# TheStageAI/TheWhisper

Hardware: NVIDIA H100
Metric: tokens_per_sec (higher is better)
Workload: dtype bf16

## Files before the change

include/thewhisper_b200.h:

```cpp
#ifndef THEWHISPER_B200_H_
#define THEWHISPER_B200_H_

#include <stddef.h>
#include <stdint.h>

#ifdef __cplusplus
extern "C" {
#endif

#define BW_ABI_VERSION 2

typedef struct bw_engine bw_engine;

#ifndef THEWHISPER_B200_TYPES_
#define THEWHISPER_B200_TYPES_
typedef struct bw_config {
  int32_t d_model;
  int32_t n_heads;
  int32_t ffn;
  int32_t enc_layers;
  int32_t dec_layers;
  int32_t n_mels;
  int32_t vocab;
  int32_t max_source_positions;
// ... 52 lines not shown
int bw_word_timestamps_batch(bw_engine* e, int32_t n, const int32_t* audio, const int32_t* n_tokens, const int32_t* num_frames,
                             double time_precision, float* out_host, int32_t out_pitch, void* stream);
int bw_word_timestamps_gather(bw_engine* e, int32_t n, const int32_t* slot_map, int32_t map_pitch, const int32_t* n_tokens,
                              const int32_t* num_frames, double time_precision, float* out_host, int32_t out_pitch, void* stream);

int bw_host_merge_overlapping(const int32_t* tokens, const int32_t* lens, int32_t n_seq, const double* ts,
                              int32_t* out_tokens, double* out_ts, int32_t* out_len);

typedef struct bw_host_vocab bw_host_vocab;
int bw_host_vocab_create(const uint8_t* bytes, const int64_t* offsets, int32_t n_vocab, const int32_t* kind, const char* language_names,
                         int32_t n_languages, int32_t timestamp_begin, int32_t render_begin, int32_t eos_id, int32_t sot_id,
                         int32_t startofprev_id, int32_t cleanup_spaces, bw_host_vocab** out);
void bw_host_vocab_destroy(bw_host_vocab* v);
int bw_host_decode_asr(bw_host_vocab* v, const int32_t* tokens, const int32_t* lens, int32_t n_out, const double* token_ts, const int32_t* ts_lens,
                       const double* strides, const uint8_t* has_stride, int32_t mode, int32_t return_language, double time_precision,
                       int32_t default_language, const char** json_out, int64_t* json_len);

int bw_op_gemm(const void* A, const void* W, int32_t M, int32_t N, int32_t K, const float* bias, float alpha, int32_t act,
               const float* residual, void* out, int32_t out_is_f32, int32_t impl, int32_t force_bn, void* stream);
int bw_op_gemm_splitk(const void* A, const void* W, int32_t M, int32_t N, int32_t K, int32_t n_valid, int32_t ksplit, int32_t force_bn,
                      float* out_partials, int32_t* ksplit_used, void* stream);
int bw_op_gemm_dec(const void* X, const void* W, int32_t Q, int32_t N, int32_t K, int32_t n_valid, int32_t want_split, float* out_partials,
                   int32_t* ksplit_used, void* stream);
int bw_op_gelu_bias(const float* partials, int32_t nsplit, const float* bias, void* h_bf16, int32_t Q, int32_t N, void* stream);
int bw_op_resid_ln(float* x, const float* partials, int32_t nsplit, const float* bias, const float* ln_g, const float* ln_b, void* y_bf16,
                   int32_t Q, int32_t D, void* stream);
int bw_op_attn_enc(const void* qkv, void* vt_scratch, void* out, int32_t B, int32_t S, int32_t H, int32_t impl, void* stream);
int bw_op_layernorm(const float* x, const float* g, const float* b, void* out, int32_t out_is_f32, int32_t rows, int32_t D,
                    void* stream);
int bw_op_gemv(const float* x, const float* ln_g, const float* ln_b, const void* W, int32_t M, int32_t N, int32_t K,
               const float* bias, float alpha, int32_t act, const float* residual, float* out, void* stream);
int bw_op_mega_plan(int32_t Q, int32_t D, int32_t ffn, int32_t num_sms, int32_t smem_optin, int32_t static_smem, int64_t* out);
int bw_op_mega_plan_w8(int32_t Q, int32_t D, int32_t ffn, int32_t num_sms, int32_t smem_optin, int32_t static_smem, int64_t* out);

#ifdef __cplusplus
}
#endif
#endif
```

thewhisper_b200/_lib.py:

```python
from __future__ import annotations

import ctypes as C
import os
from typing import Optional

_HERE = os.path.dirname(os.path.abspath(__file__))
LIB_PATH = os.path.join(_HERE, "_C", "libthewhisper_b200.so")


class BwError(RuntimeError):
    pass


class bw_config(C.Structure):
    _fields_ = [(n, C.c_int32) for n in (
        "d_model", "n_heads", "ffn", "enc_layers", "dec_layers", "n_mels", "vocab", "max_source_positions",
        "max_target_positions", "max_audios", "max_beams", "n_align_heads", "max_align_steps", "dtype")]


class bw_decode_opts(C.Structure):
    _fields_ = [
        ("begin_index", C.c_int32), ("eos_token", C.c_int32), ("pad_token", C.c_int32),
        ("timestamp_rules", C.c_int32), ("timestamp_begin", C.c_int32), ("no_timestamps_token", C.c_int32),
        ("max_initial_timestamp_index", C.c_int32),
# ... 20 lines not shown
    "bw_engine_buffer": (C.c_int, [_P, C.c_char_p, C.POINTER(_P), C.POINTER(C.c_size_t)]),
    "bw_logmel": (C.c_int, [_P, _P, _I, _I, _P, _P]),
    "bw_logmel_long": (C.c_int, [_P, _P, _I, _I, _P, _P]),
    "bw_set_mel": (C.c_int, [_P, _P, _I, _P]),
    "bw_encode": (C.c_int, [_P, _I, _P]),
    "bw_decode_begin": (C.c_int, [_P, _I, _I, _P, _I, C.POINTER(bw_decode_opts), _P]),
    "bw_decode_begin_key_start": (C.c_int, [_P, _I, _I, _P, _I, C.POINTER(bw_decode_opts), _P, _P]),
    "bw_decode_run": (C.c_int, [_P, _I, _P]),
    "bw_decode_prefill": (C.c_int, [_P, _I, _I, _P]),
    "bw_decode_kernel_launches": (C.c_longlong, [_P]),
    "bw_decode_graph_stats": (C.c_int, [_P, C.POINTER(C.c_int64)]),
    "bw_decode_read": (C.c_int, [_P, _P, _P, _P, _P]),
    "bw_decode_scores_enable": (C.c_int, [_P, _I, _I, _P]),
    "bw_decode_read_scores": (C.c_int, [_P, _P, _P, _P, _P]),
    "bw_decode_reorder": (C.c_int, [_P, _P, _P, _P]),
    "bw_decode_beam_step": (C.c_int, [_P, _P, _P, _P, _P]),
    "bw_word_timestamps": (C.c_int, [_P, _I, _I, _I, C.c_double, _P, _P]),
    "bw_word_timestamps_batch": (C.c_int, [_P, _I, _P, _P, _P, C.c_double, _P, _I, _P]),
    "bw_word_timestamps_gather": (C.c_int, [_P, _I, _P, _I, _P, _P, C.c_double, _P, _I, _P]),
    "bw_host_merge_overlapping": (C.c_int, [_P, _P, _I, _P, _P, _P, _P]),
    "bw_host_vocab_create": (C.c_int, [_P, _P, _I, _P, C.c_char_p, _I, _I, _I, _I, _I, _I, _I, _P]),
    "bw_host_vocab_destroy": (None, [_P]),
    "bw_host_decode_asr": (C.c_int, [_P, _P, _P, _I, _P, _P, _P, _P, _I, _I, C.c_double, _I, _P, _P]),
    "bw_op_gemm": (C.c_int, [_P, _P, _I, _I, _I, _P, _F, _I, _P, _P, _I, _I, _I, _P]),
    "bw_op_gemm_splitk": (C.c_int, [_P, _P, _I, _I, _I, _I, _I, _I, _P, C.POINTER(_I), _P]),
    "bw_op_gemm_dec": (C.c_int, [_P, _P, _I, _I, _I, _I, _I, _P, C.POINTER(_I), _P]),
    "bw_op_gelu_bias": (C.c_int, [_P, _I, _P, _P, _I, _I, _P]),
    "bw_op_resid_ln": (C.c_int, [_P, _P, _I, _P, _P, _P, _P, _I, _I, _P]),
    "bw_op_attn_enc": (C.c_int, [_P, _P, _P, _I, _I, _I, _I, _P]),
    "bw_op_layernorm": (C.c_int, [_P, _P, _P, _P, _I, _I, _I, _P]),
    "bw_op_gemv": (C.c_int, [_P, _P, _P, _P, _I, _I, _I, _P, _F, _I, _P, _P, _P]),
    "bw_op_mega_plan": (C.c_int, [_I, _I, _I, _I, _I, _I, C.POINTER(C.c_int64)]),
    "bw_op_mega_plan_w8": (C.c_int, [_I, _I, _I, _I, _I, _I, C.POINTER(C.c_int64)]),
}

_lib: Optional[C.CDLL] = None


def load(build_if_missing: bool = False) -> C.CDLL:
    global _lib
    if _lib is not None:
        return _lib
    if not os.path.exists(LIB_PATH):
        if build_if_missing:
            from . import build as _build

            _build.build()
        else:
            raise BwError(f"{LIB_PATH} not found: run `python -m thewhisper_b200.build` (nvcc, sm_90a). "
                          "thewhisper_b200 has no CPU fallback.")
    lib = C.CDLL(LIB_PATH)
    for name, (res, args) in SYMBOLS.items():
        fn = getattr(lib, name)
        fn.restype = res
        fn.argtypes = args
    if lib.bw_abi_version() != 2:
        raise BwError("ABI version mismatch")
    _lib = lib
    return lib


def check(rc: int) -> None:
    if rc != 0:
        msg = load().bw_last_error()
        raise BwError((msg or b"unknown error").decode("utf-8", "replace") + f" (code {rc})")

# ... 14 lines not shown
```

thewhisper_b200/csrc/abi.cu:

```cuda
#include "../../include/thewhisper_b200.h"

#define BW_RENAME_SUFFIX _bf16
#include "abi_rename.h"
#undef THEWHISPER_B200_H_
#include "../../include/thewhisper_b200.h"
#include "abi_unrename.h"
#undef BW_CAT
#undef BW_CAT2
#define BW_RENAME_SUFFIX _f16
#include "abi_rename.h"
#undef THEWHISPER_B200_H_
#include "../../include/thewhisper_b200.h"
#include "abi_unrename.h"

struct bw_engine {
  int f16;
  void* impl;
};

namespace {
thread_local int g_last_f16 = 0;
}
#define BW_B(e) reinterpret_cast<bw_engine_bf16*>((e)->impl)
#define BW_H(e) reinterpret_cast<bw_engine_f16*>((e)->impl)
// ... 108 lines not shown
  g_last_f16 = 0;
  return bw_op_gemm_dec_bf16(X, W, Q, N, K, n_valid, want_split, out_partials, ksplit_used, stream);
}
int bw_op_gelu_bias(const float* partials, int32_t nsplit, const float* bias, void* h_bf16, int32_t Q, int32_t N, void* stream) {
  g_last_f16 = 0;
  return bw_op_gelu_bias_bf16(partials, nsplit, bias, h_bf16, Q, N, stream);
}
int bw_op_resid_ln(float* x, const float* partials, int32_t nsplit, const float* bias, const float* ln_g, const float* ln_b, void* y_bf16,
                   int32_t Q, int32_t D, void* stream) {
  g_last_f16 = 0;
  return bw_op_resid_ln_bf16(x, partials, nsplit, bias, ln_g, ln_b, y_bf16, Q, D, stream);
}
int bw_op_attn_enc(const void* qkv, void* vt_scratch, void* out, int32_t B, int32_t S, int32_t H, int32_t impl, void* stream) {
  g_last_f16 = 0;
  return bw_op_attn_enc_bf16(qkv, vt_scratch, out, B, S, H, impl, stream);
}
int bw_op_layernorm(const float* x, const float* g, const float* b, void* out, int32_t out_is_f32, int32_t rows, int32_t D, void* stream) {
  g_last_f16 = 0;
  return bw_op_layernorm_bf16(x, g, b, out, out_is_f32, rows, D, stream);
}
int bw_op_gemv(const float* x, const float* ln_g, const float* ln_b, const void* W, int32_t M, int32_t N, int32_t K, const float* bias,
               float alpha, int32_t act, const float* residual, float* out, void* stream) {
  g_last_f16 = 0;
  return bw_op_gemv_bf16(x, ln_g, ln_b, W, M, N, K, bias, alpha, act, residual, out, stream);
}
int bw_op_mega_plan(int32_t Q, int32_t D, int32_t ffn, int32_t num_sms, int32_t smem_optin, int32_t static_smem, int64_t* out) {
  g_last_f16 = 0;
  return bw_op_mega_plan_bf16(Q, D, ffn, num_sms, smem_optin, static_smem, out);
}
int bw_op_mega_plan_w8(int32_t Q, int32_t D, int32_t ffn, int32_t num_sms, int32_t smem_optin, int32_t static_smem, int64_t* out) {
  g_last_f16 = 0;
  return bw_op_mega_plan_w8_bf16(Q, D, ffn, num_sms, smem_optin, static_smem, out);
}

}
```

thewhisper_b200/csrc/abi_rename.h:

```cpp
#define BW_CAT2(a, b) a##b
#define BW_CAT(a, b) BW_CAT2(a, b)
#define bw_engine BW_CAT(bw_engine, BW_RENAME_SUFFIX)
#define bw_last_error BW_CAT(bw_last_error, BW_RENAME_SUFFIX)
#define bw_abi_version BW_CAT(bw_abi_version, BW_RENAME_SUFFIX)
#define bw_device_count BW_CAT(bw_device_count, BW_RENAME_SUFFIX)
#define bw_runtime_flags BW_CAT(bw_runtime_flags, BW_RENAME_SUFFIX)
#define bw_engine_create BW_CAT(bw_engine_create, BW_RENAME_SUFFIX)
#define bw_engine_destroy BW_CAT(bw_engine_destroy, BW_RENAME_SUFFIX)
#define bw_engine_set_tensor BW_CAT(bw_engine_set_tensor, BW_RENAME_SUFFIX)
#define bw_engine_set_mel_filters BW_CAT(bw_engine_set_mel_filters, BW_RENAME_SUFFIX)
#define bw_engine_set_alignment_heads BW_CAT(bw_engine_set_alignment_heads, BW_RENAME_SUFFIX)
#define bw_engine_finalize BW_CAT(bw_engine_finalize, BW_RENAME_SUFFIX)
#define bw_engine_buffer BW_CAT(bw_engine_buffer, BW_RENAME_SUFFIX)
#define bw_logmel BW_CAT(bw_logmel, BW_RENAME_SUFFIX)
#define bw_logmel_long BW_CAT(bw_logmel_long, BW_RENAME_SUFFIX)
#define bw_set_mel BW_CAT(bw_set_mel, BW_RENAME_SUFFIX)
#define bw_encode BW_CAT(bw_encode, BW_RENAME_SUFFIX)
#define bw_decode_begin BW_CAT(bw_decode_begin, BW_RENAME_SUFFIX)
#define bw_decode_begin_key_start BW_CAT(bw_decode_begin_key_start, BW_RENAME_SUFFIX)
#define bw_decode_run BW_CAT(bw_decode_run, BW_RENAME_SUFFIX)
#define bw_decode_prefill BW_CAT(bw_decode_prefill, BW_RENAME_SUFFIX)
#define bw_decode_graph_stats BW_CAT(bw_decode_graph_stats, BW_RENAME_SUFFIX)
#define bw_decode_kernel_launches BW_CAT(bw_decode_kernel_launches, BW_RENAME_SUFFIX)
#define bw_decode_read BW_CAT(bw_decode_read, BW_RENAME_SUFFIX)
#define bw_decode_scores_enable BW_CAT(bw_decode_scores_enable, BW_RENAME_SUFFIX)
#define bw_decode_read_scores BW_CAT(bw_decode_read_scores, BW_RENAME_SUFFIX)
#define bw_decode_reorder BW_CAT(bw_decode_reorder, BW_RENAME_SUFFIX)
#define bw_decode_beam_step BW_CAT(bw_decode_beam_step, BW_RENAME_SUFFIX)
#define bw_word_timestamps BW_CAT(bw_word_timestamps, BW_RENAME_SUFFIX)
#define bw_word_timestamps_batch BW_CAT(bw_word_timestamps_batch, BW_RENAME_SUFFIX)
#define bw_op_gemm BW_CAT(bw_op_gemm, BW_RENAME_SUFFIX)
#define bw_op_gemm_splitk BW_CAT(bw_op_gemm_splitk, BW_RENAME_SUFFIX)
#define bw_op_gemm_dec BW_CAT(bw_op_gemm_dec, BW_RENAME_SUFFIX)
#define bw_op_gelu_bias BW_CAT(bw_op_gelu_bias, BW_RENAME_SUFFIX)
#define bw_op_resid_ln BW_CAT(bw_op_resid_ln, BW_RENAME_SUFFIX)
#define bw_op_attn_enc BW_CAT(bw_op_attn_enc, BW_RENAME_SUFFIX)
#define bw_op_layernorm BW_CAT(bw_op_layernorm, BW_RENAME_SUFFIX)
#define bw_op_gemv BW_CAT(bw_op_gemv, BW_RENAME_SUFFIX)
#define bw_op_mega_plan BW_CAT(bw_op_mega_plan, BW_RENAME_SUFFIX)
#define bw_op_mega_plan_w8 BW_CAT(bw_op_mega_plan_w8, BW_RENAME_SUFFIX)
#define bw_word_timestamps_gather BW_CAT(bw_word_timestamps_gather, BW_RENAME_SUFFIX)
```

thewhisper_b200/csrc/abi_unrename.h:

```cpp
#undef bw_engine
#undef bw_last_error
#undef bw_abi_version
#undef bw_device_count
#undef bw_runtime_flags
#undef bw_engine_create
#undef bw_engine_destroy
#undef bw_engine_set_tensor
#undef bw_engine_set_mel_filters
#undef bw_engine_set_alignment_heads
#undef bw_engine_finalize
#undef bw_engine_buffer
#undef bw_logmel
#undef bw_logmel_long
#undef bw_set_mel
#undef bw_encode
#undef bw_decode_begin
#undef bw_decode_begin_key_start
#undef bw_decode_run
#undef bw_decode_prefill
#undef bw_decode_kernel_launches
#undef bw_decode_graph_stats
#undef bw_decode_read
#undef bw_decode_scores_enable
#undef bw_decode_read_scores
#undef bw_decode_reorder
#undef bw_decode_beam_step
#undef bw_word_timestamps
#undef bw_word_timestamps_batch
#undef bw_op_gemm
#undef bw_op_gemm_splitk
#undef bw_op_gemm_dec
#undef bw_op_gelu_bias
#undef bw_op_resid_ln
#undef bw_op_attn_enc
#undef bw_op_layernorm
#undef bw_op_gemv
#undef bw_op_mega_plan
#undef bw_op_mega_plan_w8
#undef bw_word_timestamps_gather
#undef BW_RENAME_SUFFIX
```

thewhisper_b200/csrc/api.cu:

```cuda
#include <limits.h>
#include <stdarg.h>
#include <stdlib.h>
#include <string.h>

#include <chrono>
#include <map>
#include <string>
#include <tuple>
#include <vector>

#ifdef BW_F16
#define BW_RENAME_SUFFIX _f16
#define BW_API_NS bw_api_f16
#else
#define BW_RENAME_SUFFIX _bf16
#define BW_API_NS bw_api
#endif
#include "abi_rename.h"
#include "../../include/thewhisper_b200.h"
#include "decode.cuh"
#include "decode_mega_common.cuh"
#include "kernels.h"

namespace BW_NS {
// ... 1231 lines not shown
int bw_op_layernorm(const float* x, const float* g, const float* b, void* out, int32_t out_is_f32, int32_t rows, int32_t D, void* stream) {
  BW_CHECK(x && g && b && out, "bw_op_layernorm: null pointer");
  cudaStream_t st = static_cast<cudaStream_t>(stream);
  return out_is_f32 ? layernorm_f32(st, x, g, b, static_cast<float*>(out), rows, D)
                    : layernorm_bf16(st, x, g, b, static_cast<bf16*>(out), rows, D);
}

int bw_op_gemv(const float* x, const float* ln_g, const float* ln_b, const void* W, int32_t M, int32_t N, int32_t K, const float* bias,
               float alpha, int32_t act, const float* residual, float* out, void* stream) {
  BW_CHECK(x && W && out, "bw_op_gemv: null pointer");
  GemvArgs g;
  g.x = x; g.ldx = K; g.ln_g = ln_g; g.ln_b = ln_b; g.W = static_cast<const bf16*>(W); g.N = N; g.K = K; g.M = M;
  g.bias = bias; g.alpha = alpha; g.alpha_cols = (alpha != 1.0f) ? N : 0; g.act = act; g.residual = residual; g.out = out; g.ldo = N;
  return launch_gemv(static_cast<cudaStream_t>(stream), g);
}

static int mega_plan(int32_t Q, int32_t D, int32_t ffn, int32_t num_sms, int32_t smem_optin, int32_t static_smem, int64_t* out, int esz) {
  BW_CHECK(out && Q >= 1 && D > 0 && ffn > 0 && num_sms > 0 && smem_optin > static_smem, "bw_op_mega_plan: bad arguments");
  int p0_off = 0;
  const size_t smem = mega::mega_smem_plan(Q <= 1 ? 1 : 2, D, ffn, num_sms, true, (size_t)(smem_optin - static_smem), &p0_off, esz);
  out[0] = (int64_t)smem;
  out[1] = p0_off;
  return smem ? 0 : -3;
}

int bw_op_mega_plan(int32_t Q, int32_t D, int32_t ffn, int32_t num_sms, int32_t smem_optin, int32_t static_smem, int64_t* out) {
  return mega_plan(Q, D, ffn, num_sms, smem_optin, static_smem, out, 2);
}

int bw_op_mega_plan_w8(int32_t Q, int32_t D, int32_t ffn, int32_t num_sms, int32_t smem_optin, int32_t static_smem, int64_t* out) {
  return mega_plan(Q, D, ffn, num_sms, smem_optin, static_smem, out, 1);
}

}
```

thewhisper_b200/csrc/gemm_tc.cu:

```cuda
#include <limits.h>

#include "kernels.h"

namespace BW_NS {

namespace {

constexpr int BM = 128;
constexpr int BK = 64;
constexpr int A_STAGE_BYTES = BM * BK * 2;
constexpr int THREADS = 288;
constexpr int CONSUMER_WARPS = 8;

template <int BN>
struct Cfg {
  static constexpr int STAGES = (BN == 256) ? 4 : (BN == 128) ? 6 : 8;
  static constexpr int B_STAGE_BYTES = BN * BK * 2;
  static constexpr int SMEM_BYTES = STAGES * (A_STAGE_BYTES + B_STAGE_BYTES) + 1024  + 256 ;
};

enum { EPI_GENERIC = 0, EPI_GELU = 1 , EPI_RESID = 2 , EPI_PLAIN = 3  };

struct GemmParams {
  int B, rows, N, K;
  int rows_per_item = INT_MAX;
  int fast_gelu = 0;
  int kwrap;
  int tiles_m;
  int ksplit;
  int kper;
  long long split_stride;
  GemmEpi epi;
};

__device__ __forceinline__ void tma_load_3d(void* smem_dst, const CUtensorMap* m, uint64_t* bar, int c0, int c1, int c2) {
  asm volatile(
      "cp.async.bulk.tensor.3d.shared::cluster.global.mbarrier::complete_tx::bytes [%0], [%1, {%3, %4, %5}], [%2];" ::"r"(
          smem_u32(smem_dst)),
      "l"(reinterpret_cast<uint64_t>(m)), "r"(smem_u32(bar)), "r"(c0), "r"(c1), "r"(c2)
      : "memory");
}

__device__ __forceinline__ float gelu_as(float x) {
  const float ax = fabsf(x);
  float t;
  asm("rcp.approx.ftz.f32 %0, %1;" : "=f"(t) : "f"(fmaf(0.3275911f * 0.70710678f, ax, 1.0f)));
  float q = 0.5f * 1.061405429f;
  q = fmaf(q, t, 0.5f * -1.453152027f);
  q = fmaf(q, t, 0.5f * 1.421413741f);
  q = fmaf(q, t, 0.5f * -0.284496736f);
  q = fmaf(q, t, 0.5f * 0.254829592f);
  q = (q * t) * ex2_approx((x * -0.72134752f) * x);
  return fmaf(-ax, q, fmaxf(x, 0.f));
}

template <int BN, int MODE>
__global__ void __launch_bounds__(THREADS, 1)
gemm_tc_kernel(const __grid_constant__ CUtensorMap tmA, const __grid_constant__ CUtensorMap tmW, const GemmParams p) {
  using C = Cfg<BN>;
  extern __shared__ uint8_t smem_raw[];
  uint8_t* smem = reinterpret_cast<uint8_t*>((reinterpret_cast<uintptr_t>(smem_raw) + 1023) & ~uintptr_t(1023));
  uint8_t* sA = smem;
  uint8_t* sB = smem + C::STAGES * A_STAGE_BYTES;
  uint64_t* bars = reinterpret_cast<uint64_t*>(sB + C::STAGES * C::B_STAGE_BYTES);
  uint64_t* full = bars;
  uint64_t* empty = bars + C::STAGES;

  const int warp = threadIdx.x >> 5;
  const int lane = threadIdx.x & 31;
  const int b = blockIdx.y / p.tiles_m;
  const int t0 = (blockIdx.y % p.tiles_m) * BM;
  const int n0 = blockIdx.x * BN;
  const int nk_all = (p.K + BK - 1) / BK;
  const int kb0 = (int)blockIdx.z * p.kper;
  const int nk = min(nk_all, kb0 + p.kper) - kb0;

  if (threadIdx.x == 0) {
    for (int s = 0; s < C::STAGES; ++s) {
      mbar_init(&full[s], 1);
      mbar_init(&empty[s], CONSUMER_WARPS);
    }
    fence_mbar_init();
  }
  if (warp == CONSUMER_WARPS && lane == 0) {
    tma_prefetch_desc(&tmA);
    tma_prefetch_desc(&tmW);
  }
  __syncthreads();

// ... 6 lines not shown
      }
      pdl_wait();
      pdl_launch();
      for (int kb = 0; kb < nk; ++kb) {
        const int s = kb % C::STAGES;
        const uint32_t ph = (kb / C::STAGES) & 1;
        const int k = (kb0 + kb) * BK;
        if (kb >= npre) {
          mbar_wait_wg(&empty[s], ph ^ 1);
          mbar_arrive_expect_tx(&full[s], A_STAGE_BYTES + C::B_STAGE_BYTES);
          tma_load_2d(sB + s * C::B_STAGE_BYTES, &tmW, &full[s], k, n0);
        }
        tma_load_3d(sA + s * A_STAGE_BYTES, &tmA, &full[s], k % p.kwrap, t0 + k / p.kwrap, b);
      }
    }
  } else {
    const int g = warp >> 2;
    float acc[BN / 2];
#pragma unroll
    for (int i = 0; i < BN / 2; ++i) acc[i] = 0.f;
    for (int kb = 0; kb < nk; ++kb) {
      const int s = kb % C::STAGES;
      mbar_wait_wg(&full[s], (kb / C::STAGES) & 1);
      wg_fence();
      wg_kblock<BN>(acc, smem_u32(sA + s * A_STAGE_BYTES + g * (A_STAGE_BYTES / 2)), smem_u32(sB + s * C::B_STAGE_BYTES));
      wg_commit();
      wg_wait<1>();
      if (kb > 0 && lane == 0) mbar_arrive(&empty[(kb - 1) % C::STAGES]);
    }
    wg_wait<0>();
    wg_pin(acc);

    pdl_wait();
    const GemmEpi& e = p.epi;
    constexpr bool GEN = MODE == EPI_GENERIC;
    const bool do_alpha = GEN && e.alpha != 1.0f;
    const bool do_act = GEN ? e.act == 1 : MODE == EPI_GELU;
    const bool fast_gelu = GEN ? p.fast_gelu != 0 : true;
    const bool has_pos = GEN && e.pos != nullptr;
    const bool has_res = GEN ? e.residual != nullptr : MODE == EPI_RESID;
    const bool f32out = GEN ? e.out_f32 != nullptr : MODE == EPI_RESID;
    const int r = g * 64 + (warp & 3) * 16 + (lane >> 2);
#pragma unroll
    for (int h = 0; h < 2; ++h) {
      const int t = t0 + r + 8 * h;
      if (t >= p.rows) continue;
      const int bi = t / p.rows_per_item, ti = t - bi * p.rows_per_item;
      const long long row_off = (long long)(b + bi) * e.batch_stride + (long long)ti * e.row_stride + (long long)blockIdx.z * p.split_stride;
#pragma unroll
      for (int j = 0; j < BN / 8; ++j) {
        const int n = n0 + 8 * j + 2 * (lane & 3);
        if (n >= p.N) break;
        float f0 = acc[4 * j + 2 * h], f1 = acc[4 * j + 2 * h + 1];
        if (e.bias) {
          const float2 bb = __ldg(reinterpret_cast<const float2*>(e.bias + n));
          f0 += bb.x; f1 += bb.y;
        }
        if (do_alpha && n < e.alpha_cols) { f0 *= e.alpha; f1 *= e.alpha; }
        if (do_act) {
          if (fast_gelu) { f0 = gelu_as(f0); f1 = gelu_as(f1); }
          else { f0 = gelu_erf(f0); f1 = gelu_erf(f1); }
        }
        if (has_pos) {
          const float2 q = *reinterpret_cast<const float2*>(e.pos + (long long)t * p.N + n);
          f0 += q.x; f1 += q.y;
        }
        const long long off = row_off + (long long)(n >> 6) * e.head_stride + (n & 63);
        if (has_res) {
          const float2 q = *reinterpret_cast<const float2*>(e.residual + off);
          f0 += q.x; f1 += q.y;
        }
        if (f32out) *reinterpret_cast<float2*>(e.out_f32 + off) = make_float2(f0, f1);
        else *reinterpret_cast<uint32_t*>(e.out_bf16 + off) = pack_bf16(f0, f1);
      }
    }
  }
}

__global__ void gemm_simt_kernel(GemmA a, const bf16* __restrict__ W, GemmParams p) {
  const int n = blockIdx.x * 16 + threadIdx.x;
  const int t = (blockIdx.y % p.tiles_m) * 16 + threadIdx.y;
  const int b = blockIdx.y / p.tiles_m;
  if (n >= p.N || t >= p.rows) return;
  const bf16* ab = a.base + (long long)b * a.batch_stride;
  const bf16* w = W + (long long)n * p.K;
  float acc = 0.f;
  const int kend = (p.epi.n_valid > 0 && n >= p.epi.n_valid) ? 0 : p.K;
  for (int k = 0; k < kend; ++k) {
    const float av = e2f(ab[(long long)(t + k / p.kwrap) * a.pitch + (k % p.kwrap)]);
    acc = fmaf(av, e2f(w[k]), acc);
  }
  const GemmEpi& e = p.epi;
  const long long off = (long long)b * e.batch_stride + (long long)t * e.row_stride + (long long)(n >> 6) * e.head_stride + (n & 63);
  if (e.bias) acc += e.bias[n];
  if (n < e.alpha_cols) acc *= e.alpha;
  if (e.act == 1) acc = gelu_erf(acc);
  if (e.pos) acc += e.pos[(long long)t * p.N + n];
  if (e.residual) acc += e.residual[off];
  if (e.out_f32) e.out_f32[off] = acc;
  else e.out_bf16[off] = f2e(acc);
}

typedef CUresult (*EncodeTiledFn)(CUtensorMap*, CUtensorMapDataType, cuuint32_t, void*, const cuuint64_t*, const cuuint64_t*,
                                  const cuuint32_t*, const cuuint32_t*, CUtensorMapInterleave, CUtensorMapSwizzle,
                                  CUtensorMapL2promotion, CUtensorMapFloatOOBfill);

EncodeTiledFn get_encode_fn() {
// ... 115 lines not shown
  GemmParams p;
  p.B = B; p.rows = rows; p.N = N; p.K = K;
  p.kwrap = a.kwrap >= K ? INT_MAX : a.kwrap;
  p.tiles_m = (rows + BM - 1) / BM;
  p.epi = epi;
  {
    const int nk = K / BK;
    p.ksplit = gemm_tc_ksplit(K, ksplit);
    p.kper = (nk + p.ksplit - 1) / p.ksplit;
    p.split_stride = split_stride;
  }
  const uint64_t inner = (uint64_t)(a.kwrap >= K ? K : a.kwrap);
  CUtensorMap tmA;
  if (int rc = make_tmap_3d_bf16(&tmA, a.base, (uint64_t)B, (uint64_t)a.rows_base, inner, (uint64_t)a.pitch * 2,
                                 (uint64_t)(B > 1 ? a.batch_stride : (long long)a.rows_base * a.pitch) * 2, BM, BK))
    return rc;
  int bn = force_bn;
  if (bn == 0) {
    const long long tiles128 = (long long)((N + 127) / 128) * p.tiles_m * B;
    bn = (N % 256 == 0 && tiles128 >= 4 * device_sms()) ? 256 : 128;
    if (N < 128) bn = 64;
  }
  switch (bn) {
    case 32: return launch_tc<32>(st, tmA, W, p);
    case 64: return launch_tc<64>(st, tmA, W, p);
    case 128: return launch_tc<128>(st, tmA, W, p);
    case 256: return launch_tc<256>(st, tmA, W, p);
  }
  BW_CHECK(false, "gemm_tc: unsupported BN=%d", bn);
}

bool gemm_tc2_supported(int M, int N, int K) { return K % BK == 0 && K >= BK && (N % 256 == 0 || N % 128 == 0) && M >= 1; }

int gemm_tc2(cudaStream_t st, const bf16* A, const bf16* W, int M, int N, int K, int rows_per_item, const GemmEpi& epi, int force_bn) {
  BW_CHECK((epi.out_f32 != nullptr) != (epi.out_bf16 != nullptr), "gemm_tc2: exactly one of out_f32/out_bf16 must be set");
  BW_CHECK(gemm_tc2_supported(M, N, K), "gemm_tc2: unsupported shape M=%d N=%d K=%d", M, N, K);
  BW_CHECK(!epi.pos, "gemm_tc2: positional-table epilogue is not supported (conv stem stays on gemm_tc)");
  BW_CHECK(epi.row_stride % 8 == 0 && epi.batch_stride % 8 == 0 && epi.head_stride % 8 == 0, "gemm_tc2: output strides must be multiples of 8");
  GemmParams p;
  p.B = 1; p.rows = M; p.N = N; p.K = K;
  p.rows_per_item = rows_per_item > 0 ? rows_per_item : INT_MAX;
  p.fast_gelu = 1;
  p.kwrap = INT_MAX;
  p.tiles_m = (M + BM - 1) / BM;
  p.ksplit = 1; p.kper = K / BK; p.split_stride = 0;
  p.epi = epi;
  CUtensorMap tmA;
  if (int rc = make_tmap_3d_bf16(&tmA, A, 1, (uint64_t)M, (uint64_t)K, (uint64_t)K * 2, (uint64_t)M * K * 2, BM, BK)) return rc;
  int force_mode = -1;
  if (force_bn >= 1000) {
    force_mode = EPI_GENERIC;
    force_bn -= 1000;
  }
  int bn = force_bn;
  if (bn == 0) {
    bn = (N % 256 == 0) ? 256 : 128;
    if (bn == 256) {
      const int sms = device_sms();
      const long long t256 = (long long)p.tiles_m * (N / 256);
      const long long waves = (t256 + sms - 1) / sms;
      if (t256 * 10 < waves * sms * 8) bn = 128;
    }
  }
  BW_CHECK(bn == 128 || bn == 256, "gemm_tc2: unsupported tile width %d", bn);
  BW_CHECK(N % bn == 0, "gemm_tc2: N=%d is not a multiple of the tile width %d", N, bn);
  int mode = EPI_GENERIC;
  if (epi.alpha == 1.0f) {
    if (epi.act == 1 && !epi.residual && epi.out_bf16) mode = EPI_GELU;
    else if (epi.act == 0 && epi.residual && epi.out_f32) mode = EPI_RESID;
    else if (epi.act == 0 && !epi.residual && epi.out_bf16) mode = EPI_PLAIN;
  }
  if (force_mode >= 0) mode = force_mode;
#define BW_TC2_CASE(BNV, MODEV) \
  if (bn == BNV && mode == MODEV) return launch_tc<BNV, MODEV>(st, tmA, W, p);
  BW_TC2_CASE(256, EPI_GENERIC) BW_TC2_CASE(256, EPI_GELU) BW_TC2_CASE(256, EPI_RESID) BW_TC2_CASE(256, EPI_PLAIN)
  BW_TC2_CASE(128, EPI_GENERIC) BW_TC2_CASE(128, EPI_GELU) BW_TC2_CASE(128, EPI_RESID) BW_TC2_CASE(128, EPI_PLAIN)
#undef BW_TC2_CASE
  BW_CHECK(false, "gemm_tc2: no kernel for bn=%d mode=%d", bn, mode);
}

int gemm_simt(cudaStream_t st, const GemmA& a, const bf16* W, int B, int rows, int N, int K, const GemmEpi& epi) {
  if (int rc = check_epi(epi, N)) return rc;
  GemmParams p;
  p.B = B; p.rows = rows; p.N = N; p.K = K;
  p.kwrap = a.kwrap >= K ? INT_MAX : a.kwrap;
  p.tiles_m = (rows + 15) / 16;
  p.ksplit = 1; p.kper = 0; p.split_stride = 0;
  p.epi = epi;
  dim3 grid((N + 15) / 16, p.tiles_m * B);
  gemm_simt_kernel<<<grid, dim3(16, 16), 0, st>>>(a, W, p);
  BW_CUDA_OK(cudaGetLastError());
  return 0;
}

}
```

thewhisper_b200/csrc/kernels.h:

```cpp
#pragma once
#include "common.cuh"

namespace BW_NS {

struct GemmA {
  const bf16* base = nullptr;
  long long batch_stride = 0;
  long long pitch = 0;
  int rows_base = 0;
  int kwrap = 0x7fffffff;
};

struct GemmEpi {
  const float* bias = nullptr;
  float alpha = 1.0f;
  int alpha_cols = 0x7fffffff;
  int act = 0;
  const float* residual = nullptr;
  const float* pos = nullptr;
  float* out_f32 = nullptr;
  bf16* out_bf16 = nullptr;
  long long batch_stride = 0;
  long long row_stride = 0;
  long long head_stride = 64;
  int n_valid = 0;
};

int gemm_tc(cudaStream_t st, const GemmA& a, const bf16* W, int B, int rows, int N, int K, const GemmEpi& epi,
            int force_bn );
int gemm_tc_split(cudaStream_t st, const GemmA& a, const bf16* W, int B, int rows, int N, int K, const GemmEpi& epi, int force_bn,
                  int ksplit, long long split_stride);
int gemm_tc_ksplit(int K, int ksplit);
bool gemm_tc2_supported(int M, int N, int K);
int gemm_tc2(cudaStream_t st, const bf16* A, const bf16* W, int M, int N, int K, int rows_per_item, const GemmEpi& epi, int force_bn);
int gemm_simt(cudaStream_t st, const GemmA& a, const bf16* W, int B, int rows, int N, int K, const GemmEpi& epi);

struct DecGemmPlan {
  int QB = 16, q_tiles = 1, stages = 2, kper = 1, ksplit = 1;
  size_t smem = 0;
};
DecGemmPlan gemm_dec_plan(int Q, int N, int K, int num_sms, bool want_split, bool w8 = false);
int gemm_dec(cudaStream_t st, const bf16* X, const void* W, const float* wscale, int Q, int N, int K, int n_valid, const GemmEpi& epi,
             const DecGemmPlan& pl, long long split_stride);
int launch_gelu_bias(cudaStream_t st, const float* part, int nsplit, long long split_stride, const float* bias, bf16* h, int Q, int N);

int attn_enc_tc(cudaStream_t st, const bf16* qkv, const bf16* vt, bf16* out, int B, int S, int Spad, int H);
int attn_enc_simt(cudaStream_t st, const bf16* qkv, bf16* out, int B, int S, int H);
int transpose_v(cudaStream_t st, const bf16* qkv, bf16* vt, int B, int S, int Spad, int H);

int layernorm_bf16(cudaStream_t st, const float* x, const float* g, const float* b, bf16* y, int rows, int D);
int layernorm_f32(cudaStream_t st, const float* x, const float* g, const float* b, float* y, int rows, int D);

struct LogmelPlan;
int logmel_plan_create_from_bank(LogmelPlan** out, const float* bank , int n_mels);
void logmel_plan_destroy(LogmelPlan* p);
int logmel(cudaStream_t st, const LogmelPlan* plan, const float* pcm, int B, int n_samples, int frames, bf16* out_tm,
           float* out_f32, float* scratch, unsigned* scratch_max);
int logmel_long(cudaStream_t st, const LogmelPlan* plan, const float* pcm, int B, int n_samples, float* out_f32, unsigned* scratch_max);

}
```

Before: 845.3.

## Make tc2 GEMM persistent with ping-pong warpgroups and a shared tile planner

Replaces the one-CTA-per-tile tc2 launch with a persistent kernel capped at the SM count that loops over tiles. When there are enough 128-wide tiles and K is small, it schedules two consumer warpgroups in ping-pong so one group's epilogue overlaps the other's MMA. The epilogue is factored out and now prefetches residuals in batches, and tile selection moves into a plan function exposed through the ABI. The aims are to cut launch and tail-wave waste and hide epilogue cost, at the price of more complex barrier logic and possible load imbalance.

```diff
diff --git a/include/thewhisper_b200.h b/include/thewhisper_b200.h
--- a/include/thewhisper_b200.h
+++ b/include/thewhisper_b200.h
@@ -108,6 +108,8 @@
                const float* bias, float alpha, int32_t act, const float* residual, float* out, void* stream);
 int bw_op_mega_plan(int32_t Q, int32_t D, int32_t ffn, int32_t num_sms, int32_t smem_optin, int32_t static_smem, int64_t* out);
 int bw_op_mega_plan_w8(int32_t Q, int32_t D, int32_t ffn, int32_t num_sms, int32_t smem_optin, int32_t static_smem, int64_t* out);
+int bw_op_gemm_tc2_plan(int32_t M, int32_t N, int32_t K, int32_t num_sms, int32_t* out);
+int bw_op_gemm_tc2_tiles(int32_t M, int32_t N, int32_t K, int32_t num_sms, int32_t* out, int32_t cap);
 
 #ifdef __cplusplus
 }
diff --git a/thewhisper_b200/_lib.py b/thewhisper_b200/_lib.py
--- a/thewhisper_b200/_lib.py
+++ b/thewhisper_b200/_lib.py
@@ -76,6 +76,8 @@
     "bw_op_gemv": (C.c_int, [_P, _P, _P, _P, _I, _I, _I, _P, _F, _I, _P, _P, _P]),
     "bw_op_mega_plan": (C.c_int, [_I, _I, _I, _I, _I, _I, C.POINTER(C.c_int64)]),
     "bw_op_mega_plan_w8": (C.c_int, [_I, _I, _I, _I, _I, _I, C.POINTER(C.c_int64)]),
+    "bw_op_gemm_tc2_plan": (C.c_int, [_I, _I, _I, _I, C.POINTER(_I)]),
+    "bw_op_gemm_tc2_tiles": (C.c_int, [_I, _I, _I, _I, C.POINTER(_I), _I]),
 }
 
 _lib: Optional[C.CDLL] = None
diff --git a/thewhisper_b200/csrc/abi.cu b/thewhisper_b200/csrc/abi.cu
--- a/thewhisper_b200/csrc/abi.cu
+++ b/thewhisper_b200/csrc/abi.cu
@@ -164,5 +164,13 @@
   g_last_f16 = 0;
   return bw_op_mega_plan_w8_bf16(Q, D, ffn, num_sms, smem_optin, static_smem, out);
 }
+int bw_op_gemm_tc2_plan(int32_t M, int32_t N, int32_t K, int32_t num_sms, int32_t* out) {
+  g_last_f16 = 0;
+  return bw_op_gemm_tc2_plan_bf16(M, N, K, num_sms, out);
+}
+int bw_op_gemm_tc2_tiles(int32_t M, int32_t N, int32_t K, int32_t num_sms, int32_t* out, int32_t cap) {
+  g_last_f16 = 0;
+  return bw_op_gemm_tc2_tiles_bf16(M, N, K, num_sms, out, cap);
+}
 
 }
diff --git a/thewhisper_b200/csrc/abi_rename.h b/thewhisper_b200/csrc/abi_rename.h
--- a/thewhisper_b200/csrc/abi_rename.h
+++ b/thewhisper_b200/csrc/abi_rename.h
@@ -39,4 +39,6 @@
 #define bw_op_gemv BW_CAT(bw_op_gemv, BW_RENAME_SUFFIX)
 #define bw_op_mega_plan BW_CAT(bw_op_mega_plan, BW_RENAME_SUFFIX)
 #define bw_op_mega_plan_w8 BW_CAT(bw_op_mega_plan_w8, BW_RENAME_SUFFIX)
+#define bw_op_gemm_tc2_plan BW_CAT(bw_op_gemm_tc2_plan, BW_RENAME_SUFFIX)
+#define bw_op_gemm_tc2_tiles BW_CAT(bw_op_gemm_tc2_tiles, BW_RENAME_SUFFIX)
 #define bw_word_timestamps_gather BW_CAT(bw_word_timestamps_gather, BW_RENAME_SUFFIX)
diff --git a/thewhisper_b200/csrc/abi_unrename.h b/thewhisper_b200/csrc/abi_unrename.h
--- a/thewhisper_b200/csrc/abi_unrename.h
+++ b/thewhisper_b200/csrc/abi_unrename.h
@@ -37,5 +37,7 @@
 #undef bw_op_gemv
 #undef bw_op_mega_plan
 #undef bw_op_mega_plan_w8
+#undef bw_op_gemm_tc2_plan
+#undef bw_op_gemm_tc2_tiles
 #undef bw_word_timestamps_gather
 #undef BW_RENAME_SUFFIX
diff --git a/thewhisper_b200/csrc/api.cu b/thewhisper_b200/csrc/api.cu
--- a/thewhisper_b200/csrc/api.cu
+++ b/thewhisper_b200/csrc/api.cu
@@ -1287,4 +1287,19 @@
   return mega_plan(Q, D, ffn, num_sms, smem_optin, static_smem, out, 1);
 }
 
-}
+int bw_op_gemm_tc2_plan(int32_t M, int32_t N, int32_t K, int32_t num_sms, int32_t* out) {
+  BW_CHECK(out && num_sms > 0 && gemm_tc2_supported(M, N, K), "bw_op_gemm_tc2_plan: bad arguments (M=%d N=%d K=%d sms=%d)", M, N, K, num_sms);
+  const Tc2Plan pl = gemm_tc2_plan(M, N, K, num_sms, 0);
+  const int32_t v[7] = {pl.bm, pl.bn, pl.tiles, pl.ctas, pl.rounds, pl.idle, pl.pingpong ? 1 : 0};
+  for (int i = 0; i < 7; ++i) out[i] = v[i];
+  return 0;
+}
+
+int bw_op_gemm_tc2_tiles(int32_t M, int32_t N, int32_t K, int32_t num_sms, int32_t* out, int32_t cap) {
+  BW_CHECK(out && num_sms > 0 && gemm_tc2_supported(M, N, K), "bw_op_gemm_tc2_tiles: bad arguments (M=%d N=%d K=%d sms=%d)", M, N, K, num_sms);
+  const Tc2Plan pl = gemm_tc2_plan(M, N, K, num_sms, 0);
+  BW_CHECK(cap >= pl.tiles, "bw_op_gemm_tc2_tiles: %d tiles, room for %d", pl.tiles, cap);
+  return gemm_tc2_tiles(pl, out) == pl.tiles ? 0 : -1;
+}
+
+}
diff --git a/thewhisper_b200/csrc/gemm_tc.cu b/thewhisper_b200/csrc/gemm_tc.cu
--- a/thewhisper_b200/csrc/gemm_tc.cu
+++ b/thewhisper_b200/csrc/gemm_tc.cu
@@ -55,6 +55,71 @@
 }
 
 template <int BN, int MODE>
+__device__ __forceinline__ void epilogue(const float (&acc)[BN / 2], const GemmParams& p, int b, int t_first, int n0, int lane,
+                                         long long split_off) {
+  const GemmEpi& e = p.epi;
+  constexpr bool GEN = MODE == EPI_GENERIC;
+  const bool do_alpha = GEN && e.alpha != 1.0f;
+  const bool do_act = GEN ? e.act == 1 : MODE == EPI_GELU;
+  const bool fast_gelu = GEN ? p.fast_gelu != 0 : true;
+  const bool has_pos = GEN && e.pos != nullptr;
+  const bool has_res = GEN ? e.residual != nullptr : MODE == EPI_RESID;
+  const bool f32out = GEN ? e.out_f32 != nullptr : MODE == EPI_RESID;
+#pragma unroll
+  for (int h = 0; h < 2; ++h) {
+    const int t = t_first + 8 * h;
+    if (t >= p.rows) continue;
+    const int bi = t / p.rows_per_item, ti = t - bi * p.rows_per_item;
+    const long long row_off = (long long)(b + bi) * e.batch_stride + (long long)ti * e.row_stride + split_off;
+    constexpr int RJ = MODE == EPI_RESID ? (BN / 8 < 8 ? BN / 8 : 8) : BN / 8;
+#pragma unroll
+    for (int j0 = 0; j0 < BN / 8; j0 += RJ) {
+      float2 res[MODE == EPI_RESID ? RJ : 1];
+      if (MODE == EPI_RESID) {
+#pragma unroll
+        for (int jj = 0; jj < RJ; ++jj) {
+          const int n = n0 + 8 * (j0 + jj) + 2 * (lane & 3);
+          if (n >= p.N) break;
+          res[jj] = *reinterpret_cast<const float2*>(e.residual + row_off + (long long)(n >> 6) * e.head_stride + (n & 63));
+        }
+      }
+#pragma unroll
+      for (int jj = 0; jj < RJ; ++jj) {
+        const int j = j0 + jj;
+        const int n = n0 + 8 * j + 2 * (lane & 3);
+        if (n >= p.N) break;
+        float f0 = acc[4 * j + 2 * h], f1 = acc[4 * j + 2 * h + 1];
+        if (e.bias) {
+          const float2 bb = __ldg(reinterpret_cast<const float2*>(e.bias + n));
+          f0 += bb.x; f1 += bb.y;
+        }
+        if (do_alpha && n < e.alpha_cols) { f0 *= e.alpha; f1 *= e.alpha; }
+        if (do_act) {
+          if (fast_gelu) { f0 = gelu_as(f0); f1 = gelu_as(f1); }
+          else { f0 = gelu_erf(f0); f1 = gelu_erf(f1); }
+        }
+        if (has_pos) {
+          const float2 q = *reinterpret_cast<const float2*>(e.pos + (long long)t * p.N + n);
+          f0 += q.x; f1 += q.y;
+        }
+        const long long off = row_off + (long long)(n >> 6) * e.head_stride + (n & 63);
+        if (has_res) {
+          const float2 q = MODE == EPI_RESID ? res[MODE == EPI_RESID ? jj : 0] : *reinterpret_cast<const float2*>(e.residual + off);
+          f0 += q.x; f1 += q.y;
+        }
+        if (f32out) *reinterpret_cast<float2*>(e.out_f32 + off) = make_float2(f0, f1);
+        else *reinterpret_cast<uint32_t*>(e.out_bf16 + off) = pack_bf16(f0, f1);
+      }
+    }
+  }
+}
+
+__host__ __device__ __forceinline__ void tc2_tile(int tile, int tiles_n, int bn, int* m0, int* n0) {
+  *m0 = (tile / tiles_n) * BM;
+  *n0 = (tile % tiles_n) * bn;
+}
+
+template <int BN, int MODE>
 __global__ void __launch_bounds__(THREADS, 1)
 gemm_tc_kernel(const __grid_constant__ CUtensorMap tmA, const __grid_constant__ CUtensorMap tmW, const GemmParams p) {
   using C = Cfg<BN>;
@@ -127,47 +192,104 @@
     wg_pin(acc);
 
     pdl_wait();
-    const GemmEpi& e = p.epi;
-    constexpr bool GEN = MODE == EPI_GENERIC;
-    const bool do_alpha = GEN && e.alpha != 1.0f;
-    const bool do_act = GEN ? e.act == 1 : MODE == EPI_GELU;
-    const bool fast_gelu = GEN ? p.fast_gelu != 0 : true;
-    const bool has_pos = GEN && e.pos != nullptr;
-    const bool has_res = GEN ? e.residual != nullptr : MODE == EPI_RESID;
-    const bool f32out = GEN ? e.out_f32 != nullptr : MODE == EPI_RESID;
-    const int r = g * 64 + (warp & 3) * 16 + (lane >> 2);
-#pragma unroll
-    for (int h = 0; h < 2; ++h) {
-      const int t = t0 + r + 8 * h;
-      if (t >= p.rows) continue;
-      const int bi = t / p.rows_per_item, ti = t - bi * p.rows_per_item;
-      const long long row_off = (long long)(b + bi) * e.batch_stride + (long long)ti * e.row_stride + (long long)blockIdx.z * p.split_stride;
-#pragma unroll
-      for (int j = 0; j < BN / 8; ++j) {
-        const int n = n0 + 8 * j + 2 * (lane & 3);
-        if (n >= p.N) break;
-        float f0 = acc[4 * j + 2 * h], f1 = acc[4 * j + 2 * h + 1];
-        if (e.bias) {
-          const float2 bb = __ldg(reinterpret_cast<const float2*>(e.bias + n));
-          f0 += bb.x; f1 += bb.y;
-        }
-        if (do_alpha && n < e.alpha_cols) { f0 *= e.alpha; f1 *= e.alpha; }
-        if (do_act) {
-          if (fast_gelu) { f0 = gelu_as(f0); f1 = gelu_as(f1); }
-          else { f0 = gelu_erf(f0); f1 = gelu_erf(f1); }
-        }
-        if (has_pos) {
-          const float2 q = *reinterpret_cast<const float2*>(e.pos + (long long)t * p.N + n);
-          f0 += q.x; f1 += q.y;
-        }
-        const long long off = row_off + (long long)(n >> 6) * e.head_stride + (n & 63);
-        if (has_res) {
-          const float2 q = *reinterpret_cast<const float2*>(e.residual + off);
-          f0 += q.x; f1 += q.y;
-        }
-        if (f32out) *reinterpret_cast<float2*>(e.out_f32 + off) = make_float2(f0, f1);
-        else *reinterpret_cast<uint32_t*>(e.out_bf16 + off) = pack_bf16(f0, f1);
-      }
+    epilogue<BN, MODE>(acc, p, b, t0 + g * 64 + (warp & 3) * 16 + (lane >> 2), n0, lane, (long long)blockIdx.z * p.split_stride);
+  }
+}
+
+template <int BN, bool PP, int MODE>
+__global__ void __launch_bounds__(THREADS, 1)
+gemm_tc2_kernel(const __grid_constant__ CUtensorMap tmA, const __grid_constant__ CUtensorMap tmW, const GemmParams p) {
+  using C = Cfg<BN>;
+  static_assert(!PP || BN == 128, "ping-pong holds a whole 128 x BN tile per warpgroup: BN = 128 only");
+  constexpr int NACC = PP ? 2 : 1;
+  extern __shared__ uint8_t smem_raw[];
+  uint8_t* smem = reinterpret_cast<uint8_t*>((reinterpret_cast<uintptr_t>(smem_raw) + 1023) & ~uintptr_t(1023));
+  uint8_t* sA = smem;
+  uint8_t* sB = smem + C::STAGES * A_STAGE_BYTES;
+  uint64_t* bars = reinterpret_cast<uint64_t*>(sB + C::STAGES * C::B_STAGE_BYTES);
+  uint64_t* full = bars;
+  uint64_t* empty = bars + C::STAGES;
+  uint64_t* issued = bars + 2 * C::STAGES;
+
+  const int warp = threadIdx.x >> 5;
+  const int lane = threadIdx.x & 31;
+  const int tiles_n = p.N / BN;
+  const int ntiles = p.tiles_m * tiles_n;
+  const int nk = p.K / BK;
+
+  if (threadIdx.x == 0) {
+    for (int s = 0; s < C::STAGES; ++s) {
+      mbar_init(&full[s], 1);
+      mbar_init(&empty[s], PP ? CONSUMER_WARPS / 2 : CONSUMER_WARPS);
+    }
+    mbar_init(&issued[0], CONSUMER_WARPS / 2);
+    mbar_init(&issued[1], CONSUMER_WARPS / 2);
+    fence_mbar_init();
+  }
+  if (warp == CONSUMER_WARPS && lane == 0) {
+    tma_prefetch_desc(&tmA);
+    tma_prefetch_desc(&tmW);
+  }
+  __syncthreads();
+
+  if (warp == CONSUMER_WARPS) {
+    if (lane == 0) {
+      int m0, n0;
+      tc2_tile(blockIdx.x, tiles_n, BN, &m0, &n0);
+      const int npre = nk < C::STAGES ? nk : C::STAGES;
+      for (int kb = 0; kb < npre; ++kb) {
+        mbar_arrive_expect_tx(&full[kb], A_STAGE_BYTES + C::B_STAGE_BYTES);
+        tma_load_2d(sB + kb * C::B_STAGE_BYTES, &tmW, &full[kb], kb * BK, n0);
+      }
+      pdl_wait();
+      pdl_launch();
+      int it = 0;
+      for (int tile = blockIdx.x; tile < ntiles; tile += gridDim.x) {
+        tc2_tile(tile, tiles_n, BN, &m0, &n0);
+        for (int kb = 0; kb < nk; ++kb, ++it) {
+          const int s = it % C::STAGES;
+          if (it >= npre) {
+            mbar_wait_wg(&empty[s], ((it / C::STAGES) & 1) ^ 1);
+            mbar_arrive_expect_tx(&full[s], A_STAGE_BYTES + C::B_STAGE_BYTES);
+            tma_load_2d(sB + s * C::B_STAGE_BYTES, &tmW, &full[s], kb * BK, n0);
+          }
+          tma_load_3d(sA + s * A_STAGE_BYTES, &tmA, &full[s], kb * BK, m0, 0);
+        }
+      }
+    }
+  } else {
+    const int g = warp >> 2;
+    float acc[NACC][BN / 2];
+    for (int j = PP ? g : 0, tile = blockIdx.x + j * gridDim.x; tile < ntiles; j += PP ? 2 : 1, tile += (PP ? 2 : 1) * gridDim.x) {
+      int m0, n0;
+      tc2_tile(tile, tiles_n, BN, &m0, &n0);
+      if (PP && j > 0) mbar_wait_wg(&issued[g ^ 1], ((j - 1) >> 1) & 1);
+#pragma unroll
+      for (int a = 0; a < NACC; ++a)
+#pragma unroll
+        for (int i = 0; i < BN / 2; ++i) acc[a][i] = 0.f;
+      const int row0 = PP ? 0 : g * 64;
+      for (int kb = 0; kb < nk; ++kb) {
+        const int it = j * nk + kb;
+        const int s = it % C::STAGES;
+        mbar_wait_wg(&full[s], (it / C::STAGES) & 1);
+        wg_fence();
+#pragma unroll
+        for (int a = 0; a < NACC; ++a)
+          wg_kblock<BN>(acc[a], smem_u32(sA + s * A_STAGE_BYTES + (row0 + 64 * a) * (BK * 2)), smem_u32(sB + s * C::B_STAGE_BYTES));
+        wg_commit();
+        wg_wait<1>();
+        if (kb > 0 && lane == 0) mbar_arrive(&empty[(it - 1) % C::STAGES]);
+      }
+      if (PP && lane == 0) mbar_arrive(&issued[g]);
+      wg_wait<0>();
+#pragma unroll
+      for (int a = 0; a < NACC; ++a) wg_pin(acc[a]);
+      if (lane == 0) mbar_arrive(&empty[(j * nk + nk - 1) % C::STAGES]);
+
+      pdl_wait();
+#pragma unroll
+      for (int a = 0; a < NACC; ++a) epilogue<BN, MODE>(acc[a], p, 0, m0 + row0 + 64 * a + (warp & 3) * 16 + (lane >> 2), n0, lane, 0);
     }
   }
 }
@@ -349,10 +471,61 @@
 
 bool gemm_tc2_supported(int M, int N, int K) { return K % BK == 0 && K >= BK && (N % 256 == 0 || N % 128 == 0) && M >= 1; }
 
+Tc2Plan gemm_tc2_plan(int M, int N, int K, int sms, int force_bn) {
+  Tc2Plan pl;
+  pl.bm = BM;
+  pl.tiles_m = (M + BM - 1) / BM;
+  int bn = force_bn;
+  if (bn == 0) {
+    bn = (N % 256 == 0) ? 256 : 128;
+    if (bn == 256) {
+      const long long t256 = (long long)pl.tiles_m * (N / 256);
+      const long long rounds = (t256 + sms - 1) / sms;
+      if (t256 * 10 < rounds * sms * 8) bn = 128;
+    }
+  }
+  const long long t128 = (long long)pl.tiles_m * (N / 128);
+  pl.pingpong = (force_bn == 0 || force_bn == 128) && K <= 2048 && t128 >= 2LL * sms;
+  if (pl.pingpong) bn = 128;
+  pl.bn = bn;
+  pl.tiles_n = N / bn;
+  pl.tiles = pl.tiles_m * pl.tiles_n;
+  pl.ctas = pl.tiles < sms ? pl.tiles : sms;
+  pl.rounds = (pl.tiles + pl.ctas - 1) / pl.ctas;
+  pl.idle = pl.rounds * pl.ctas - pl.tiles;
+  return pl;
+}
+
+int gemm_tc2_tiles(const Tc2Plan& pl, int32_t* out) {
+  int k = 0;
+  for (int c = 0; c < pl.ctas; ++c)
+    for (int tile = c; tile < pl.tiles; tile += pl.ctas, ++k) {
+      int m0, n0;
+      tc2_tile(tile, pl.tiles_n, pl.bn, &m0, &n0);
+      out[3 * k] = c; out[3 * k + 1] = m0; out[3 * k + 2] = n0;
+    }
+  return k;
+}
+
+template <int BN, bool PP, int MODE>
+static int launch_tc2(cudaStream_t st, const CUtensorMap& tmA, const bf16* W, const GemmParams& p, int ctas) {
+  using C = Cfg<BN>;
+  CUtensorMap tmW;
+  if (int rc = make_tmap_2d_bf16(&tmW, W, p.N, p.K, (uint64_t)p.K * 2, BN, BK)) return rc;
+  static bool attr_set = false;
+  if (!attr_set) {
+    BW_CUDA_OK(cudaFuncSetAttribute(gemm_tc2_kernel<BN, PP, MODE>, cudaFuncAttributeMaxDynamicSharedMemorySize, C::SMEM_BYTES));
+    attr_set = true;
+  }
+  BW_CUDA_OK(launch_k(gemm_tc2_kernel<BN, PP, MODE>, dim3(ctas), dim3(THREADS), (size_t)C::SMEM_BYTES, st, tmA, tmW, p));
+  return 0;
+}
+
 int gemm_tc2(cudaStream_t st, const bf16* A, const bf16* W, int M, int N, int K, int rows_per_item, const GemmEpi& epi, int force_bn) {
   BW_CHECK((epi.out_f32 != nullptr) != (epi.out_bf16 != nullptr), "gemm_tc2: exactly one of out_f32/out_bf16 must be set");
   BW_CHECK(gemm_tc2_supported(M, N, K), "gemm_tc2: unsupported shape M=%d N=%d K=%d", M, N, K);
   BW_CHECK(!epi.pos, "gemm_tc2: positional-table epilogue is not supported (conv stem stays on gemm_tc)");
+  BW_CHECK(epi.n_valid == 0 || epi.n_valid == N, "gemm_tc2: every row of W must exist (n_valid=%d, N=%d)", epi.n_valid, N);
   BW_CHECK(epi.row_stride % 8 == 0 && epi.batch_stride % 8 == 0 && epi.head_stride % 8 == 0, "gemm_tc2: output strides must be multiples of 8");
   GemmParams p;
   p.B = 1; p.rows = M; p.N = N; p.K = K;
@@ -369,17 +542,9 @@
     force_mode = EPI_GENERIC;
     force_bn -= 1000;
   }
-  int bn = force_bn;
-  if (bn == 0) {
-    bn = (N % 256 == 0) ? 256 : 128;
-    if (bn == 256) {
-      const int sms = device_sms();
-      const long long t256 = (long long)p.tiles_m * (N / 256);
-      const long long waves = (t256 + sms - 1) / sms;
-      if (t256 * 10 < waves * sms * 8) bn = 128;
-    }
-  }
-  BW_CHECK(bn == 128 || bn == 256, "gemm_tc2: unsupported tile width %d", bn);
+  BW_CHECK(force_bn == 0 || force_bn == 128 || force_bn == 256, "gemm_tc2: unsupported tile width %d", force_bn);
+  const Tc2Plan pl = gemm_tc2_plan(M, N, K, device_sms(), force_bn);
+  const int bn = pl.bn;
   BW_CHECK(N % bn == 0, "gemm_tc2: N=%d is not a multiple of the tile width %d", N, bn);
   int mode = EPI_GENERIC;
   if (epi.alpha == 1.0f) {
@@ -388,10 +553,11 @@
     else if (epi.act == 0 && !epi.residual && epi.out_bf16) mode = EPI_PLAIN;
   }
   if (force_mode >= 0) mode = force_mode;
-#define BW_TC2_CASE(BNV, MODEV) \
-  if (bn == BNV && mode == MODEV) return launch_tc<BNV, MODEV>(st, tmA, W, p);
-  BW_TC2_CASE(256, EPI_GENERIC) BW_TC2_CASE(256, EPI_GELU) BW_TC2_CASE(256, EPI_RESID) BW_TC2_CASE(256, EPI_PLAIN)
-  BW_TC2_CASE(128, EPI_GENERIC) BW_TC2_CASE(128, EPI_GELU) BW_TC2_CASE(128, EPI_RESID) BW_TC2_CASE(128, EPI_PLAIN)
+#define BW_TC2_CASE(BNV, PPV, MODEV) \
+  if (bn == BNV && pl.pingpong == PPV && mode == MODEV) return launch_tc2<BNV, PPV, MODEV>(st, tmA, W, p, pl.ctas);
+  BW_TC2_CASE(256, false, EPI_GENERIC) BW_TC2_CASE(256, false, EPI_GELU) BW_TC2_CASE(256, false, EPI_RESID) BW_TC2_CASE(256, false, EPI_PLAIN)
+  BW_TC2_CASE(128, false, EPI_GENERIC) BW_TC2_CASE(128, false, EPI_GELU) BW_TC2_CASE(128, false, EPI_RESID) BW_TC2_CASE(128, false, EPI_PLAIN)
+  BW_TC2_CASE(128, true, EPI_GENERIC) BW_TC2_CASE(128, true, EPI_GELU) BW_TC2_CASE(128, true, EPI_RESID) BW_TC2_CASE(128, true, EPI_PLAIN)
 #undef BW_TC2_CASE
   BW_CHECK(false, "gemm_tc2: no kernel for bn=%d mode=%d", bn, mode);
 }
diff --git a/thewhisper_b200/csrc/kernels.h b/thewhisper_b200/csrc/kernels.h
--- a/thewhisper_b200/csrc/kernels.h
+++ b/thewhisper_b200/csrc/kernels.h
@@ -33,6 +33,12 @@
 int gemm_tc_ksplit(int K, int ksplit);
 bool gemm_tc2_supported(int M, int N, int K);
 int gemm_tc2(cudaStream_t st, const bf16* A, const bf16* W, int M, int N, int K, int rows_per_item, const GemmEpi& epi, int force_bn);
+struct Tc2Plan {
+  int bm, bn, tiles_m, tiles_n, tiles, ctas, rounds, idle;
+  bool pingpong;
+};
+Tc2Plan gemm_tc2_plan(int M, int N, int K, int sms, int force_bn);
+int gemm_tc2_tiles(const Tc2Plan& pl, int32_t* out);
 int gemm_simt(cudaStream_t st, const GemmA& a, const bf16* W, int B, int rows, int N, int K, const GemmEpi& epi);
 
 struct DecGemmPlan {
```

Result: no change. 847.6, median of 6 (+0.3%).
